# tum-vision/dvo_slam

Hardware: NVIDIA H100
Metric: frame-pair alignments/sec @640x480x5-level (higher is better)
Workload: dtype f32

## Files before the change

### dvo_slam_b200/csrc/capi.cu

```cuda
#include "common.cuh"

#include <cstdio>
#include <cstdlib>
#include <cstring>
#include <limits>
#include <vector>

namespace dvo_b200 {

int set_error(dvo_b200_ctx* ctx, int code, const std::string& msg) {
  if (ctx) ctx->last_error = msg;
  return code;
}

int check_cuda(dvo_b200_ctx* ctx, cudaError_t e, const char* what) {
  if (e == cudaSuccess) return 0;
  std::string msg = std::string("CUDA error: ") + cudaGetErrorString(e) + " in " + what;
  cudaGetLastError();
  return set_error(ctx, e == cudaErrorMemoryAllocation ? DVO_B200_ERR_OUT_OF_MEMORY : DVO_B200_ERR_CUDA, msg);
}

static cudaEvent_t get_event(dvo_b200_ctx* ctx) {
  if (!ctx->event_pool.empty()) { cudaEvent_t e = ctx->event_pool.back(); ctx->event_pool.pop_back(); return e; }
  cudaEvent_t e;
// ... 50 lines not shown
  if (cudaGetDeviceCount(&count) != cudaSuccess || count <= 0 || device < 0 || device >= count) {
    cudaGetLastError();
    return DVO_B200_ERR_CUDA;
  }
  if (cudaSetDevice(device) != cudaSuccess) { cudaGetLastError(); return DVO_B200_ERR_CUDA; }
  dvo_b200_ctx* ctx = new dvo_b200_ctx;
  ctx->device = device;
  ctx->pool = std::make_shared<SlabPool>();
  ctx->pool->device = device;
  if (stream) { ctx->stream = (cudaStream_t)stream; ctx->own_stream = false; }
  else {
    if (cudaStreamCreateWithFlags(&ctx->stream, cudaStreamNonBlocking) != cudaSuccess) { cudaGetLastError(); delete ctx; return DVO_B200_ERR_CUDA; }
    ctx->own_stream = true;
  }
  if (getenv("DVO_B200_TIMING")) {
    cudaMalloc((void**)&ctx->d_dbg, sizeof(unsigned long long) * 256);
    cudaMemset(ctx->d_dbg, 0, sizeof(unsigned long long) * 256);
    for (int l = 0; l < 8; ++l) { unsigned long long big = ~0ull; cudaMemcpy(ctx->d_dbg + 128 + 8 * l + 6, &big, 8, cudaMemcpyHostToDevice); }
  }
  *out = ctx;
  return 0;
}

int dvo_b200_destroy(dvo_b200_ctx* ctx) {
  if (!ctx) return DVO_B200_ERR_INVALID_ARGUMENT;
  cudaSetDevice(ctx->device);
  cudaStreamSynchronize(ctx->stream);
  drain_profile(ctx);
  for (cudaEvent_t e : ctx->event_pool) cudaEventDestroy(e);
  Workspace& ws = ctx->ws;
  cudaFree(ws.d_pair_level); cudaFree(ws.d_state); cudaFree(ws.d_row_exports); cudaFree(ws.d_row_base);
  cudaFree(ws.d_strip_exports); cudaFree(ws.d_strip_base); cudaFree(ws.d_row_partial); cudaFree(ws.d_strip_partial); cudaFree(ws.d_dump); cudaFree(ws.d_tinit);
// ... 234 lines not shown
  return tracker_linearize(ctx, cfg, reference, current, level, T, use_weights, prev_precision, count, precision_out, ll_out,
                           A_out, b_out, nullptr);
}

int dvo_b200_profile_enable(dvo_b200_ctx* ctx, int32_t enable) {
  if (!ctx) return DVO_B200_ERR_INVALID_ARGUMENT;
  ctx->profile = enable != 0;
  return 0;
}

int dvo_b200_profile_read(dvo_b200_ctx* ctx, double ms_out[8], int64_t launches_out[8], int32_t reset) {
  if (!ctx) return DVO_B200_ERR_INVALID_ARGUMENT;
  cudaSetDevice(ctx->device);
  drain_profile(ctx);
  if (ctx->d_dbg) {
    unsigned long long h[256];
    cudaStreamSynchronize(ctx->stream);
    cudaMemcpy(h, ctx->d_dbg, sizeof(h), cudaMemcpyDeviceToHost);
    static const char* names[8] = {"stageA", "stageB", "waitA", "waitB", "mid", "end", "queue", "total"};
    for (int l = 0; l < 8; ++l) {
      const unsigned long long* v = h + 16 * l;
      if (!v[7]) continue;
      fprintf(stderr, "[dvo_b200 timing] level-slot %d:", l);
      for (int i = 0; i < 8; ++i) fprintf(stderr, " %s=%.1f%%", names[i], 100.0 * (double)v[i] / (double)v[7]);
      fprintf(stderr, " (cta-ms total %.1f)\n", (double)v[7] * 1e-6);
      fprintf(stderr, "[dvo_b200 timing]   consumer warp 0: wait-full %.1f%% of stage A, %.1f%% of stage B; producer: descriptor %.1f%%, "
                      "wait-empty %.1f%% of its stage time\n", 100.0 * (double)v[9] / (double)(v[8] + 1), 100.0 * (double)v[11] / (double)(v[10] + 1),
              100.0 * (double)v[12] / (double)(v[14] + v[15] + 1), 100.0 * (double)v[13] / (double)(v[14] + v[15] + 1));
      const unsigned long long* u = h + 128 + 8 * l;
      if (u[0]) fprintf(stderr, "[dvo_b200 timing]   tiles %llu (inexact %.2f%%, skipped %.2f%%), stage-B rounds in the generic loop %.2f%%; CTA lifetime of the last launch-set: "
                                "max %.3f ms, min %.3f ms\n", u[0], 100.0 * (double)u[1] / (double)u[0], 100.0 * (double)u[2] / (double)u[0],
                        100.0 * (double)u[4] / (double)(u[3] + 1), (double)u[5] * 1e-6, (double)u[6] * 1e-6);
      const unsigned long long* e = h + 192 + 8 * l;
      if (e[7]) {
        double tot = 0;
        for (int i = 0; i < 6; ++i) tot += (double)e[i];
        fprintf(stderr, "[dvo_b200 timing]   end step: critical part %.1f%% of the end time; of the end thread's time: partial sums %.1f%%, state+log %.1f%%, "
                        "LDLT %.1f%%, exp+K*T %.1f%%, release %.1f%%, deferred %.1f%% (total %.1f cta-ms)\n", 100.0 * (double)e[7] / (double)(v[5] + 1),
                100.0 * e[0] / tot, 100.0 * e[1] / tot, 100.0 * e[2] / tot, 100.0 * e[3] / tot, 100.0 * e[4] / tot, 100.0 * e[5] / tot, tot * 1e-6);
      }
    }
    if (reset) {
      cudaMemset(ctx->d_dbg, 0, sizeof(h));
      for (int l = 0; l < 8; ++l) { unsigned long long big = ~0ull; cudaMemcpy(ctx->d_dbg + 128 + 8 * l + 6, &big, 8, cudaMemcpyHostToDevice); }
    }
  }
  if (getenv("DVO_B200_TIMING")) {
// ... 15 lines not shown
```

### dvo_slam_b200/csrc/stages.cuh

```cuda
#pragma once
#include "common.cuh"
#include "f32x2.cuh"

namespace dvo_b200 {

constexpr unsigned kFullMask = 0xffffffffu;
constexpr int kConsumerWarps = kTileH;
constexpr int kCtaThreads = (kConsumerWarps + 1) * 32;
#ifndef DVO_WIN_COLS
#define DVO_WIN_COLS 152
#endif
#ifndef DVO_WIN_ROWS
#define DVO_WIN_ROWS 24
#endif
#ifndef DVO_STAGES
#define DVO_STAGES 2
#endif
constexpr int kWinCols = DVO_WIN_COLS;
constexpr int kWinRows = DVO_WIN_ROWS;
constexpr int kStages = DVO_STAGES;

__device__ __forceinline__ unsigned smem_u32(const void* p) { return (unsigned)__cvta_generic_to_shared(p); }
__device__ __forceinline__ void mbar_init(unsigned long long* bar, unsigned count) {
  asm volatile("mbarrier.init.shared::cta.b64 [%0], %1;" ::"r"(smem_u32(bar)), "r"(count) : "memory");
}
__device__ __forceinline__ void mbar_fence_init() { asm volatile("fence.mbarrier_init.release.cluster;" ::: "memory"); }
__device__ __forceinline__ void mbar_arrive(unsigned long long* bar) {
  asm volatile("{\n\t.reg .b64 st;\n\tmbarrier.arrive.release.cta.shared::cta.b64 st, [%0];\n\t}" ::"r"(smem_u32(bar)) : "memory");
}
__device__ __forceinline__ void mbar_arrive_expect_tx(unsigned long long* bar, unsigned bytes) {
  asm volatile("{\n\t.reg .b64 st;\n\tmbarrier.arrive.expect_tx.release.cta.shared::cta.b64 st, [%0], %1;\n\t}" ::"r"(smem_u32(bar)),
               "r"(bytes)
               : "memory");
}
#ifndef DVO_TRYWAIT_HINT_NS
// ... 48 lines not shown
    if (((++spins) & 0xfffu) == 0u) {
      if (*reinterpret_cast<volatile int*>(error_flag)) break;
      if (spins > (1u << 24)) { atomicExch(error_flag, 2); break; }
    }
  }
}
__device__ __forceinline__ void mbar_arrive_s(unsigned bar) {
  asm volatile("{\n\t.reg .b64 st;\n\tmbarrier.arrive.release.cta.shared::cta.b64 st, [%0];\n\t}" ::"r"(bar) : "memory");
}
__device__ __forceinline__ int4 lds_i4(unsigned addr) {
  int4 v;
  asm volatile("ld.shared.v4.b32 {%0, %1, %2, %3}, [%4];" : "=r"(v.x), "=r"(v.y), "=r"(v.z), "=r"(v.w) : "r"(addr));
  return v;
}

__device__ __forceinline__ void bulk_g2s(void* dst_smem, const void* src_gmem, unsigned bytes, unsigned long long* bar) {
  asm volatile("cp.async.bulk.shared::cta.global.mbarrier::complete_tx::bytes [%0], [%1], %2, [%3];" ::"r"(smem_u32(dst_smem)),
               "l"(src_gmem), "r"(bytes), "r"(smem_u32(bar))
               : "memory");
}

template <int kOff>
__device__ __forceinline__ f2 lds_f2(unsigned addr) {
  f2 v;
  asm volatile("ld.shared.v2.f32 {%0, %1}, [%2+%3];" : "=f"(v.x), "=f"(v.y) : "r"(addr), "n"(kOff));
  return v;
}
__device__ __forceinline__ float lds_f32(unsigned addr) {
  float v;
  asm volatile("ld.shared.f32 %0, [%1];" : "=f"(v) : "r"(addr));
// ... 15 lines not shown
  int skip;
  int origin;
  int ulo, ucount;
  int vlo, vcount;
  int exact;
  int pad_;
};
struct __align__(128) StageBuf {
  float2 ref0[kTileH][kTileW];
  float tx[kTileW];
  float2 ref1[kTileH][kTileW];
  float2 win[kWinRows][kWinCols];
};
static_assert(offsetof(StageBuf, tx) == kRecTx * sizeof(float2) && offsetof(StageBuf, ref1) == kRecP1 * sizeof(float2) &&
              offsetof(StageBuf, win) == kRecF2 * sizeof(float2), "StageBuf must mirror the reference tile record");
struct TilePipe {
  StageBuf buf[kStages];
  unsigned long long full[kStages], empty[kStages];
  TileDesc desc[kStages];
};
static_assert(sizeof(TileDesc) == 32 && offsetof(TilePipe, desc) % 16 == 0, "TileDesc is read as two 16-byte words");

#ifdef DVO_PIPE_TIMING
struct PipeTiming {
  unsigned long long wait_full_a = 0, wait_full_b = 0, wait_empty = 0, produce = 0, rounds_a = 0, rounds_b = 0;
  unsigned long long tiles = 0, tiles_inexact = 0, tiles_skipped = 0, slow_rounds = 0, rounds = 0;
  bool on = false;
};
#define DVO_CLOCK(tm) ((tm).on ? clock64() : 0)
#define DVO_ADD(tm, field, v) do { if ((tm).on) (tm).field += (v); } while (0)
#else
struct PipeTiming {};
#define DVO_CLOCK(tm) 0ll
#define DVO_ADD(tm, field, v) do { } while (0)
#endif

struct LevelGeom {
  int w, h, n, pitch;
  int nbands, nstrips;
  int strip0, strip_step, nmine;
};
// ... 17 lines not shown
  c.k0 = pk(kt[0], kt[4]); c.k1 = pk(kt[1], kt[5]); c.k2 = pk(kt[2], kt[6]); c.k3 = pk(kt[3], kt[7]);
  c.k8 = kt[8]; c.k9 = kt[9]; c.k10 = kt[10]; c.k11 = kt[11];
  c.Pa = pk(P[0], P[1]); c.Pb = pk(P[2], P[3]);
  const float cgx = __fdiv_rn(__fmul_rn(0.5f, pl.cfx), 255.0f), cgy = __fdiv_rn(__fmul_rn(0.5f, pl.cfy), 255.0f);
  c.cg = pk(cgx, cgy);
  c.cgh = pk(0.5f * cgx, 0.5f * cgy);
  c.fxyh = pk(0.5f * pl.cfx, 0.5f * pl.cfy);
  c.c_i = 1.0f / 255.0f;
  c.ubx = pin((float)(w - 2)); c.uby = pin((float)(h - 2));
  c.first_iteration = __ldcg(&st.iteration) == 0;
}

template <bool kStageB>
__device__ __noinline__ void produce_tiles(TilePipe& tp, const PairLevel& pl, const LevelGeom& g, const StageConsts& c, unsigned tbase,
                                           int ntiles, int* error_flag, PipeTiming& tm) {
  const int lane = threadIdx.x & 31, sub = lane >> 3;
  const float2* cur = kStageB ? pl.c3 : pl.c0;
  int s_issue = g.strip0, b_issue = 0;
  for (int i0 = 0; i0 < ntiles; i0 += 4) {
    const long long tp0 = DVO_CLOCK(tm);
    unsigned wordA, wordD;
    {
      const int ii = min(i0 + sub, ntiles - 1);
      const int sd = ii / g.nbands;
      const int s = g.strip0 + sd * g.strip_step, b = ii - sd * g.nbands;
      const int y0 = s * kTileH, rows = min(kTileH, g.h - y0);
      const int x0 = b * kTileW, bw = min(kTileW, g.w - x0);
      const float2 zr = __ldg(pl.rrange + (size_t)s * g.nbands + b);
      const float txc = __ldg(pl.rtmpl + ((lane & 1) ? x0 + bw - 1 : x0));
      const float tyc = __ldg(pl.rtmpl + g.w + ((lane & 2) ? y0 + rows - 1 : y0));
      const bool has_depth = zr.x <= zr.y;
      const float z = (lane & 4) ? zr.y : zr.x;
      const float px = txc * z, py = tyc * z;
// ... 4 lines not shown
      const bool front_lane = Zt > 1e-6f && umin == umin && vmin == vmin;
#pragma unroll
      for (int off = 1; off < 8; off <<= 1) {
        umin = fminf(umin, __shfl_xor_sync(kFullMask, umin, off)); umax = fmaxf(umax, __shfl_xor_sync(kFullMask, umax, off));
        vmin = fminf(vmin, __shfl_xor_sync(kFullMask, vmin, off)); vmax = fmaxf(vmax, __shfl_xor_sync(kFullMask, vmax, off));
      }
      const bool front = ((__ballot_sync(kFullMask, front_lane) >> (sub * 8)) & 0xffu) == 0xffu;
      umin = fmaxf(umin, -8.f); vmin = fmaxf(vmin, -8.f); umax = fminf(umax, (float)g.w + 8.f); vmax = fminf(vmax, (float)g.h + 8.f);
      int skip = 0, exact = 0, ncols = 0, nrows = 0, bx0 = 0, row_lo = 0;
      if (!has_depth) {
        skip = 1;
      } else if (!front) {
      } else if (umax < -1.f || vmax < -1.f || umin > (float)g.w || vmin > (float)g.h) {
        skip = 1;
      } else {
        const int col_lo = max((int)floorf(umin) - 2, 0), col_hi = min((int)floorf(umax) + 3, g.w - 1);
        row_lo = max((int)floorf(vmin) - 2, -1);
        const int row_hi = min((int)floorf(vmax) + 3, g.h);
        bx0 = col_lo & ~1;
        ncols = (col_hi + 2 - bx0) & ~1;
        bool whole = true;
        if (ncols > kWinCols) { bx0 += ((ncols - kWinCols) / 2) & ~1; ncols = kWinCols; whole = false; }
        nrows = row_hi - row_lo + 1;
        if (nrows > kWinRows) { row_lo += (nrows - kWinRows) / 2; nrows = kWinRows; whole = false; }
        if (ncols < 4 || nrows < 4) { ncols = 0; nrows = 0; bx0 = 0; row_lo = 0; }
        else exact = whole ? 1 : 0;
      }
      wordA = (unsigned)skip | ((unsigned)exact << 1) | ((unsigned)ncols << 2) | ((unsigned)nrows << 10);
      wordD = (unsigned)bx0 | ((unsigned)(row_lo + 1) << 16);
    }
    DVO_ADD(tm, produce, DVO_CLOCK(tm) - tp0);
    const int kmax = min(4, ntiles - i0);
    for (int k = 0; k < kmax; ++k) {
      const unsigned t = tbase + (unsigned)(i0 + k);
      const int bufi = t % kStages;
      StageBuf& sb = tp.buf[bufi];
      const unsigned wa = __shfl_sync(kFullMask, wordA, k * 8), wd = __shfl_sync(kFullMask, wordD, k * 8);
      const int s = s_issue, b = b_issue;
      if (++b_issue == g.nbands) { b_issue = 0; s_issue += g.strip_step; }
      const int skip = (int)(wa & 1u), ncols = (int)((wa >> 2) & 0xffu), nrows = (int)(wa >> 10);
      const int win_bx0 = (int)(wd & 0xffffu), win_row_lo = (int)(wd >> 16) - 1;
      TileDesc d;
      d.skip = skip; d.exact = (int)((wa >> 1) & 1u); d.pad_ = 0;
      d.origin = 0; d.ulo = 0; d.ucount = 0; d.vlo = 0; d.vcount = 0;
      if (ncols) {
        d.origin = (win_row_lo * kWinCols + win_bx0) * 8;
        d.ulo = win_bx0 == 0 ? 0 : win_bx0 + 1;
        const int uhi = (win_bx0 + ncols - 1 >= g.w - 1) ? g.w - 2 : win_bx0 + ncols - 3;
        d.ucount = max(uhi - d.ulo + 1, 0);
        d.vlo = win_row_lo + 1;
        d.vcount = max(nrows - 3, 0);
      }
      const unsigned win_row_bytes = (unsigned)ncols * 8u;
      const unsigned rec_bytes = (unsigned)(kStageB ? kRecF2 : kRecP1) * 8u;
      const unsigned total = skip ? 0u : rec_bytes + (unsigned)nrows * win_row_bytes;
      const long long tp1 = DVO_CLOCK(tm);
      mbar_wait(&tp.empty[bufi], ((t / kStages) & 1u) ^ 1u, error_flag);
      DVO_ADD(tm, wait_empty, DVO_CLOCK(tm) - tp1);
      DVO_ADD(tm, tiles, 1); DVO_ADD(tm, tiles_inexact, (!d.skip && !d.exact) ? 1 : 0); DVO_ADD(tm, tiles_skipped, d.skip ? 1 : 0);
      if (lane == 0) {
        tp.desc[bufi] = d;
        if (total) mbar_arrive_expect_tx(&tp.full[bufi], total);
        else mbar_arrive(&tp.full[bufi]);
      }
      __syncwarp();
      if (!skip) {
        if (lane < nrows) {
          const int yy = min(max(win_row_lo + lane, 0), g.h - 1);
          bulk_g2s(&sb.win[lane][0], cur + (size_t)yy * g.pitch + win_bx0, win_row_bytes, &tp.full[bufi]);
        }
        if (lane == 31) bulk_g2s(&sb.ref0[0][0], pl.r0 + (size_t)(s * g.nbands + b) * kRecF2, rec_bytes, &tp.full[bufi]);
      }
    }
  }
}

struct PixelProjection {
  f2 f, gq;
  float Zt;
  int u0, v0;
  bool inb;
};

__device__ __forceinline__ PixelProjection project_pixel(float tx, float ty, float z, const StageConsts& c) {
  PixelProjection p;
  const f2 pxy = mul2(pk(tx, ty), bc(z));
// ... 344 lines not shown
  }
  if (lane == 0) {
    seg_out[0] = __int_as_float(st.cnt);
    seg_out[1] = (float)(0.5 * ((double)all0 + (double)alt0)); seg_out[2] = (float)(0.5 * ((double)all1 + (double)alt1));
    seg_out[3] = (float)(0.5 * ((double)all2 + (double)alt2));
    seg_out[4] = (float)(0.5 * ((double)all0 - (double)alt0)); seg_out[5] = (float)(0.5 * ((double)all1 - (double)alt1));
    seg_out[6] = (float)(0.5 * ((double)all2 - (double)alt2));
    seg_out[7] = st.wfirst;
    if (st.cnt == 0) { seg_out[8] = 0.f; seg_out[9] = 0.f; seg_out[10] = 0.f; seg_out[11] = 0.f; }
  }
  if (st.pend) {
    seg_out[8] = st.pw; seg_out[9] = st.po0; seg_out[10] = st.po1; seg_out[11] = st.po2;
  }
}

__device__ __forceinline__ WinView make_view(unsigned bufs, const int4& d0, const int4& d1, const float2* plane, int w, int h, int pitch) {
  WinView wv;
  const unsigned w0 = bufs + (unsigned)offsetof(StageBuf, win);
  wv.base = pin(w0 - (unsigned)d0.y);
  wv.safe = pin(w0 + (unsigned)((kWinCols + 1) * 8));
  wv.plane = plane;
  wv.exact = d1.z != 0;
  wv.ulo = d0.z; wv.ucount = d0.w; wv.vlo = d1.x; wv.vcount = d1.y;
  wv.w = w; wv.h = h; wv.pitch = pitch;
  return wv;
}


template <bool kCorrected, bool kExact, bool kFirst>
__device__ __forceinline__ void stage_a_rounds(const WinView& wv, int bw, unsigned refa, unsigned txa, float ty, const StageConsts& c,
                                               typename ScaleOf<kCorrected>::type& ss, int lane, unsigned lt_mask, int odd_col,
                                               float odd_z) {
  static_assert(kTileW % 64 == 0, "the exact loop takes whole pairs of rounds");
// ... 15 lines not shown
      z0 = (r * 32 + lane == odd_col) ? odd_z : z0;
      z1 = (r * 32 + 32 + lane == odd_col) ? odd_z : z1;
    }
    const PixelProjection p0 = project_pixel(tx0, ty, z0, c);
    const PixelProjection p1 = project_pixel(tx1, ty, z1, c);
    float ei0, ez0, ei1, ez1;
    const bool v0 = residual_pixel<kExact>(p0, wv, lo(rz0), z0, c, ei0, ez0);
    const bool v1 = residual_pixel<kExact>(p1, wv, lo(rz1), z1, c, ei1, ez1);
    const float w0 = student_weight(c, first, ei0, ez0), w1 = student_weight(c, first, ei1, ez1);
    scale_add(ss, lane, lt_mask, v0, w0, ei0, ez0);
    scale_add(ss, lane, lt_mask, v1, w1, ei1, ez1);
  }
}
template <bool kCorrected>
__device__ __forceinline__ void stage_a_run(TilePipe& tp, const PairLevel& pl, const LevelGeom& g, const StageConsts& c,
                                            float* row_exports, unsigned& tile_count, int* error_flag, PipeTiming& tm) {
  const int lane = threadIdx.x & 31, q = threadIdx.x >> 5;
  const unsigned lt_mask = (1u << lane) - 1u;
  const int ntiles = g.nmine * g.nbands;
  const unsigned tbase = tile_count;
  tile_count += ntiles;
  if (q == kConsumerWarps) {
    produce_tiles<false>(tp, pl, g, c, tbase, ntiles, error_flag, tm);
    return;
  }
  int i = 0;
  const unsigned tp_s = pin(smem_u32(&tp));
  const unsigned my_ref = pin((unsigned)(offsetof(StageBuf, ref0) + (q * kTileW + lane) * 8));
  const unsigned my_tx = pin((unsigned)(offsetof(StageBuf, tx) + lane * 4));
  const int gw = pin(g.w), gh = pin(g.h), gnb = pin(g.nbands), gpitch = g.pitch;
  OddPoint odd;
  odd.y = -1; odd.x = 0; odd.z = 0.f;
  if (kCorrected) odd = load_odd_point(pl, g);
  for (int sk = 0, s = g.strip0; sk < g.nmine; ++sk, s += g.strip_step) {
    const int y = s * kTileH + q;
    const bool row_ok = y < gh;
    const float ty = __ldg(pl.rtmpl + gw + min(y, gh - 1));
    typename ScaleOf<kCorrected>::type ss;
    scale_state_init(ss);
    for (int b = 0; b < gnb; ++b, ++i) {
      const unsigned t = tbase + i;
      const unsigned bufi = t % kStages;
      const int x0 = b * kTileW, bw = min(kTileW, gw - x0);
      const long long tw0 = DVO_CLOCK(tm);
      mbar_wait_s(tp_s + (unsigned)offsetof(TilePipe, full) + bufi * 8u, (t / kStages) & 1u, error_flag);
      DVO_ADD(tm, wait_full_a, DVO_CLOCK(tm) - tw0);
      const unsigned bufs = tp_s + bufi * (unsigned)sizeof(StageBuf);
      const int4 d0 = lds_i4(tp_s + (unsigned)offsetof(TilePipe, desc) + bufi * 32u);
      if (row_ok && !d0.x) {
        const int4 d1 = lds_i4(tp_s + (unsigned)offsetof(TilePipe, desc) + bufi * 32u + 16u);
        const WinView wv = make_view(bufs, d0, d1, pl.c0, gw, gh, gpitch);
        const unsigned refa = bufs + my_ref, txa = bufs + my_tx;
        const bool odd_tile = kCorrected && y == odd.y && (unsigned)(odd.x - x0) < (unsigned)bw;
        if (wv.exact && bw == kTileW && !odd_tile) {
          if (c.first_iteration) stage_a_rounds<kCorrected, true, true>(wv, bw, refa, txa, ty, c, ss, lane, lt_mask, -1, 0.f);
          else stage_a_rounds<kCorrected, true, false>(wv, bw, refa, txa, ty, c, ss, lane, lt_mask, -1, 0.f);
        } else {
          stage_a_rounds<kCorrected, false, false>(wv, bw, refa, txa, ty, c, ss, lane, lt_mask, odd_tile ? odd.x - x0 : -1, odd.z);
        }
      }
      __syncwarp();
      if (lane == 0) mbar_arrive_s(tp_s + (unsigned)offsetof(TilePipe, empty) + bufi * 8u);
    }
    if (row_ok) scale_state_export(ss, lane, row_exports + (size_t)y * kSegExportFloats);
  }
}

struct StageBConsts {
  float P00, P01, P10, P11;
  float l, wd0, wd1;
};

constexpr int kNormalValues = 28;

constexpr int kTriValues = 21;
__host__ __device__ constexpr int tri(int r, int c) { return r * 6 - r * (r - 1) / 2 + (c - r); }
struct StageBAcc {
// ... 118 lines not shown
      const unsigned m = __ballot_sync(kFullMask, valid);
      keep = valid && (rank + __popc(m & lt_mask)) < keep_rank;
      rank += __popc(m);
    }
    if (kDump && r * 32 < xlim) dump_record(dump, pix + r * 32, valid, E, G, H, z);
    const float ei = valid ? lo(E) : 0.f, ez = valid ? hi(E) : 0.f;
    const float wall = student_weight(c, first, ei, ez);
    const float wgt = valid ? wall : 0.f;
    stage_b_pixel(acc, cb, wgt, keep, ei, ez, valid ? G : bc(0.f), valid ? H : bc(0.f), valid ? z : 1.0f, valid ? tx : 0.f, ty);
  }
}

template <bool kDump, bool kCorrected>
__device__ __forceinline__ void stage_b_run(TilePipe& tp, const PairLevel& pl, const LevelGeom& g, const StageConsts& c,
                                            const StageBConsts& cb, const int* row_base, const int* strip_base, long long n_keep,
                                            const RecordDump& dump, float* row_partial, unsigned& tile_count, int* error_flag,
                                            PipeTiming& tm) {
  const int lane = threadIdx.x & 31, q = threadIdx.x >> 5;
  const unsigned lt_mask = (1u << lane) - 1u;
  const int ntiles = g.nmine * g.nbands;
  const unsigned tbase = tile_count;
  tile_count += ntiles;
  if (q == kConsumerWarps) {
    produce_tiles<true>(tp, pl, g, c, tbase, ntiles, error_flag, tm);
    return;
  }
  int i = 0;
  const unsigned tp_s = pin(smem_u32(&tp));
  const unsigned my_ref = (unsigned)(offsetof(StageBuf, ref0) + (q * kTileW + lane) * 8);
  const unsigned my_tx = (unsigned)(offsetof(StageBuf, tx) + lane * 4);
  const int gw = g.w, gh = g.h, gnb = g.nbands, gpitch = g.pitch;
  OddPoint odd;
  odd.y = -1; odd.x = 0; odd.z = 0.f;
  if (kCorrected) odd = load_odd_point(pl, g);
  for (int sk = 0, s = g.strip0; sk < g.nmine; ++sk, s += g.strip_step) {
    const int y = s * kTileH + q;
    const bool row_ok = y < gh;
// ... 2 lines not shown
    int keep_rank = 0;
    int rank = 0;
    if (!kCorrected) {
      const long long sbase = __ldcg(strip_base + s);
      cta_has_tail = (long long)__ldcg(strip_base + s + 1) > n_keep;
      keep_rank = (int)max(min(n_keep - sbase, (long long)0x7fffffff), (long long)-1);
      if (cta_has_tail && row_ok) rank = __ldcg(row_base + y);
    }
    StageBAcc acc;
    stage_b_init(acc);
    for (int b = 0; b < gnb; ++b, ++i) {
      const unsigned t = tbase + i;
      const unsigned bufi = t % kStages;
      const int x0 = b * kTileW, bw = min(kTileW, gw - x0);
      const long long tw0 = DVO_CLOCK(tm);
      mbar_wait_s(tp_s + (unsigned)offsetof(TilePipe, full) + bufi * 8u, (t / kStages) & 1u, error_flag);
      DVO_ADD(tm, wait_full_b, DVO_CLOCK(tm) - tw0);
      const unsigned bufs = tp_s + bufi * (unsigned)sizeof(StageBuf);
      const int4 d0 = lds_i4(tp_s + (unsigned)offsetof(TilePipe, desc) + bufi * 32u);
      if (row_ok && !d0.x) {
        const int4 d1 = lds_i4(tp_s + (unsigned)offsetof(TilePipe, desc) + bufi * 32u + 16u);
        const WinView wv = make_view(bufs, d0, d1, pl.c3, gw, gh, gpitch);
        const unsigned refa = bufs + my_ref, txa = bufs + my_tx;
        const size_t pix = (size_t)y * gw + x0 + lane;
        const bool odd_tile = kCorrected && y == odd.y && (unsigned)(odd.x - x0) < (unsigned)bw;
        if (wv.exact && bw == kTileW && !cta_has_tail && !odd_tile) {
          if (c.first_iteration)
            stage_b_rounds<kCorrected, true, true, kDump>(wv, bw, refa, txa, ty, c, cb, acc, cta_has_tail, rank, keep_rank, dump, pix, lane,
                                                          lt_mask, -1, 0.f, tm);
          else
            stage_b_rounds<kCorrected, true, false, kDump>(wv, bw, refa, txa, ty, c, cb, acc, cta_has_tail, rank, keep_rank, dump, pix, lane,
                                                           lt_mask, -1, 0.f, tm);
        } else {
          stage_b_rounds<kCorrected, false, false, kDump>(wv, bw, refa, txa, ty, c, cb, acc, cta_has_tail, rank, keep_rank, dump, pix, lane,
                                                          lt_mask, odd_tile ? odd.x - x0 : -1, odd.z, tm);
        }
      } else if (kDump && row_ok) {
        for (int xl = lane; xl < bw; xl += 32) dump_record(dump, (size_t)y * gw + x0 + xl, false, bc(0.f), bc(0.f), bc(0.f), 0.f);
      }
      __syncwarp();
      if (lane == 0) mbar_arrive_s(tp_s + (unsigned)offsetof(TilePipe, empty) + bufi * 8u);
    }
    if (row_ok) flush_row_partial(acc, lane, row_partial + (size_t)y * kNormalValues);
  }
}

__device__ __forceinline__ void load_stage_b_consts(const PairState& st, StageBConsts& c) {
  c.P00 = __ldcg(&st.precision[0]); c.P01 = __ldcg(&st.precision[1]); c.P10 = __ldcg(&st.precision[2]); c.P11 = __ldcg(&st.precision[3]);
  c.l = c.P01 / c.P00;
  c.wd0 = c.P00;
  c.wd1 = c.P11 - c.P01 * c.l;
}

}
```

### dvo_slam_b200/csrc/tracker.cu

```cuda
#include "common.cuh"
#include "stages.cuh"

#include <cstdio>
#include <cstring>
#include <limits>
#include <cmath>
#include <cstdlib>
#include <algorithm>

namespace dvo_b200 {

namespace {

constexpr unsigned kFull = 0xffffffffu;
constexpr int kEndWarps = 4;

struct LevelLaunch {
  int w, h, n, pitch;
  int nbands, nstrips;
  int level_index;
  int level_id;
  int max_iterations;
  int first_level;
  int use_initial_estimate;
// ... 252 lines not shown
}

struct SquadState {
  int pair;
  unsigned arrive;
  unsigned phase;
  int pad_[29];
};

struct LevelTail {
  SegCombineSmem comb;
  PairEndSmem end;
  int s_flag[2];
};
constexpr size_t kLevelSmemBytes = sizeof(TilePipe) + sizeof(LevelTail);

constexpr int kMaxSeg = 4;
struct Segment {
  const PairLevel* pls;
  float* row_exports;
  int* row_base;
  double* strip_exports;
  int* strip_base;
  float* row_partial;
  double* strip_partial;
  SquadState* squads;
  int* queue;
  int* ready;
  int* ready_tail;
  int* arrivals;
// ... 61 lines not shown
    }
  }
  __syncthreads();
}

template <bool kCorrected>
__global__ void __launch_bounds__(kCtaThreads, 2)
k_level_persistent(const __grid_constant__ PersistentArgs a) {
  extern __shared__ __align__(128) unsigned char smem_raw[];
  TilePipe& tp = *reinterpret_cast<TilePipe*>(smem_raw);
  LevelTail& lt = *reinterpret_cast<LevelTail*>(smem_raw + sizeof(TilePipe));

  const int warp = threadIdx.x >> 5, lane = threadIdx.x & 31;

  if (threadIdx.x == 0) {
    for (int i = 0; i < kStages; ++i) { mbar_init(&tp.full[i], 1); mbar_init(&tp.empty[i], kConsumerWarps); }
    mbar_fence_init();
  }
  __syncthreads();
  unsigned tile_count = 0;
  const bool fused = a.nseg >= 2;
#define DVO_TICK() do { if (timing) t0 = global_ns(); } while (0)
#define DVO_TOCK(slot) do { if (timing) { t1 = global_ns(); t_acc[slot] += t1 - t0; t0 = t1; } } while (0)

#pragma unroll 1
  for (int si = 0; si < a.nseg; ++si) {
  const Segment& S = a.seg[si];
  int cta_index = blockIdx.x;
  if (fused && si >= 1) {
    if (threadIdx.x == 0) lt.s_flag[1] = atomicAdd(S.arrivals, 1);
    __syncthreads();
    cta_index = lt.s_flag[1];
    __syncthreads();
  }
  const int squad = cta_index / S.g, rank = cta_index - squad * S.g;
// ... 68 lines not shown
          squad_release(sq, episode);
        }
      } else {
        squad_wait(sq, episode, a.error_flag);
      }
      __syncthreads();
      ++episode;
      DVO_TOCK(6);
    }

    for (;;) {
      {
        StageConsts c;
        load_stage_consts(st, pl, lp.w, lp.h, false, c);
        const long long ts0 = DVO_CLOCK(tm);
        stage_a_run<kCorrected>(tp, pl, geo, c, row_exports, tile_count, a.error_flag, tm);
        DVO_ADD(tm, rounds_a, DVO_CLOCK(tm) - ts0);
      }
      __syncthreads();
      for (int j = threadIdx.x; j < geo.nmine; j += kCtaThreads) {
        const int sj = geo.strip0 + j * geo.strip_step;
        combine_strip_rows(row_exports, sj * kTileH, min(sj * kTileH + kTileH, lp.h), row_base, strip_exports + (size_t)sj * kStripExportDoubles);
      }
      DVO_TOCK(0);
      if (squad_arrive(sq, episode, S.g, lt.s_flag)) {
        DVO_TOCK(2);
        if (warp == 0) {
          pair_mid_warp<kCorrected>(st, pair, strip_exports, strip_base, lp.nstrips, nullptr, lp, a.ilog, a.max_log, lt.comb);
          if (lane == 0) squad_release(sq, episode);
        }
        __syncthreads();
// ... 3 lines not shown
        DVO_TOCK(2);
      }
      __syncthreads();
      ++episode;
      if (!__ldcg(&st.level_active) || *reinterpret_cast<volatile int*>(a.error_flag)) break;

      {
        StageConsts c;
        load_stage_consts(st, pl, lp.w, lp.h, true, c);
        StageBConsts cb;
        load_stage_b_consts(st, cb);
        const long long n_keep = __ldcg(&st.n_keep);
        RecordDump dump;
        dump.planes = a.dump; dump.n = lp.n;
        const long long ts0 = DVO_CLOCK(tm);
        if (a.dump) stage_b_run<true, kCorrected>(tp, pl, geo, c, cb, row_base, strip_base, n_keep, dump, row_partial, tile_count, a.error_flag, tm);
        else stage_b_run<false, kCorrected>(tp, pl, geo, c, cb, row_base, strip_base, n_keep, dump, row_partial, tile_count, a.error_flag, tm);
        DVO_ADD(tm, rounds_b, DVO_CLOCK(tm) - ts0);
      }
      __syncthreads();
      for (int it = threadIdx.x; it < geo.nmine * kNormalValues; it += kCtaThreads) {
        const int j = it / kNormalValues, i = it - j * kNormalValues;
        const int sj = geo.strip0 + j * geo.strip_step;
        const int nrow = min(kTileH, lp.h - sj * kTileH);
        const float* rp = row_partial + (size_t)sj * kTileH * kNormalValues + i;
        float r[kTileH];
#pragma unroll
        for (int k = 0; k < kTileH; ++k) r[k] = k < nrow ? __ldcg(rp + (size_t)k * kNormalValues) : 0.f;
        double v = 0.0;
#pragma unroll
        for (int k = 0; k < kTileH; ++k) v += (double)r[k];
        strip_partial[(size_t)sj * kNormalValues + i] = v;
// ... 20 lines not shown
      __threadfence();
      const int slot = atomicAdd(a.seg[k].ready_tail, 1);
      asm volatile("st.release.gpu.global.u32 [%0], %1;" :: "l"(a.seg[k].ready + slot), "r"(pair + 1) : "memory");
    }
  }
  if (timing) {
    t_acc[7] = global_ns() - t_start;
    for (int i = 0; i < 8; ++i) atomicAdd(S.dbg + i, t_acc[i]);
  }
#ifdef DVO_PIPE_TIMING
  if (tm.on) {
    if (warp == 0) { atomicAdd(S.dbg + 8, tm.rounds_a); atomicAdd(S.dbg + 9, tm.wait_full_a); atomicAdd(S.dbg + 10, tm.rounds_b); atomicAdd(S.dbg + 11, tm.wait_full_b); }
    else { atomicAdd(S.dbg + 12, tm.produce); atomicAdd(S.dbg + 13, tm.wait_empty); atomicAdd(S.dbg + 14, tm.rounds_a); atomicAdd(S.dbg + 15, tm.rounds_b); }
    if (warp == 0) { atomicAdd(S.dbg2 + 3, tm.rounds); atomicAdd(S.dbg2 + 4, tm.slow_rounds); }
    else { atomicAdd(S.dbg2 + 0, tm.tiles); atomicAdd(S.dbg2 + 1, tm.tiles_inexact); atomicAdd(S.dbg2 + 2, tm.tiles_skipped); }
  }
  if (timing) { atomicMax(S.dbg2 + 5, t_acc[7]); atomicMin(S.dbg2 + 6, t_acc[7]); }
#endif
  }
#undef DVO_TICK
#undef DVO_TOCK
}

__global__ void k_finalize(PairState* states, dvo_b200_result* results, int npairs) {
  int p = blockIdx.x * blockDim.x + threadIdx.x;
  if (p >= npairs) return;
  PairState& st = states[p];
  dvo_b200_result& r = results[p];
  const double nan = __longlong_as_double(0x7ff8000000000000LL);
  se3_matrix(se3_inverse(st.estimate), r.transformation);
// ... 560 lines not shown
```

Measured before the change: 21140.

## Give stage A its own smaller-window, deeper tile ring sharing stage B's smem

Splits the tile pipeline into separate stage-A and stage-B rings that share one shared-memory union. Stage A gets a 16-row window with no third gradient record, a tighter halo and three slots, so its producer can prefetch further ahead. Stage B keeps its 2-slot, 24-row layout. Each stage now has its own barriers, descriptors and tile counters, and a proxy fence is added before the bulk copies reuse the slots. The change also adds timing counters for stage A, and any stage-A tile whose footprint exceeds 16 rows falls off the exact path more often.

```diff
diff --git a/dvo_slam_b200/csrc/capi.cu b/dvo_slam_b200/csrc/capi.cu
--- a/dvo_slam_b200/csrc/capi.cu
+++ b/dvo_slam_b200/csrc/capi.cu
@@ -88,8 +88,8 @@
     ctx->own_stream = true;
   }
   if (getenv("DVO_B200_TIMING")) {
-    cudaMalloc((void**)&ctx->d_dbg, sizeof(unsigned long long) * 256);
-    cudaMemset(ctx->d_dbg, 0, sizeof(unsigned long long) * 256);
+    cudaMalloc((void**)&ctx->d_dbg, sizeof(unsigned long long) * 320);
+    cudaMemset(ctx->d_dbg, 0, sizeof(unsigned long long) * 320);
     for (int l = 0; l < 8; ++l) { unsigned long long big = ~0ull; cudaMemcpy(ctx->d_dbg + 128 + 8 * l + 6, &big, 8, cudaMemcpyHostToDevice); }
   }
   *out = ctx;
@@ -354,7 +354,7 @@
   cudaSetDevice(ctx->device);
   drain_profile(ctx);
   if (ctx->d_dbg) {
-    unsigned long long h[256];
+    unsigned long long h[320];
     cudaStreamSynchronize(ctx->stream);
     cudaMemcpy(h, ctx->d_dbg, sizeof(h), cudaMemcpyDeviceToHost);
     static const char* names[8] = {"stageA", "stageB", "waitA", "waitB", "mid", "end", "queue", "total"};
@@ -371,6 +371,10 @@
       if (u[0]) fprintf(stderr, "[dvo_b200 timing]   tiles %llu (inexact %.2f%%, skipped %.2f%%), stage-B rounds in the generic loop %.2f%%; CTA lifetime of the last launch-set: "
                                 "max %.3f ms, min %.3f ms\n", u[0], 100.0 * (double)u[1] / (double)u[0], 100.0 * (double)u[2] / (double)u[0],
                         100.0 * (double)u[4] / (double)(u[3] + 1), (double)u[5] * 1e-6, (double)u[6] * 1e-6);
+      const unsigned long long* a = h + 256 + 8 * l;
+      if (a[1]) fprintf(stderr, "[dvo_b200 timing]   stage A: tiles %llu (inexact %.2f%%, skipped %.2f%%), producer wait-empty %.1f%% of its stage-A time; "
+                                "stage B: producer wait-empty %.1f%% of its stage-B time\n", a[1], 100.0 * (double)a[2] / (double)a[1],
+                        100.0 * (double)a[3] / (double)a[1], 100.0 * (double)a[0] / (double)(v[14] + 1), 100.0 * (double)(v[13] - a[0]) / (double)(v[15] + 1));
       const unsigned long long* e = h + 192 + 8 * l;
       if (e[7]) {
         double tot = 0;
diff --git a/dvo_slam_b200/csrc/stages.cuh b/dvo_slam_b200/csrc/stages.cuh
--- a/dvo_slam_b200/csrc/stages.cuh
+++ b/dvo_slam_b200/csrc/stages.cuh
@@ -16,9 +16,17 @@
 #ifndef DVO_STAGES
 #define DVO_STAGES 2
 #endif
+#ifndef DVO_WIN_ROWS_A
+#define DVO_WIN_ROWS_A 16
+#endif
+#ifndef DVO_STAGES_A
+#define DVO_STAGES_A 3
+#endif
 constexpr int kWinCols = DVO_WIN_COLS;
 constexpr int kWinRows = DVO_WIN_ROWS;
 constexpr int kStages = DVO_STAGES;
+constexpr int kWinRowsA = DVO_WIN_ROWS_A;
+constexpr int kStagesA = DVO_STAGES_A;
 
 __device__ __forceinline__ unsigned smem_u32(const void* p) { return (unsigned)__cvta_generic_to_shared(p); }
 __device__ __forceinline__ void mbar_init(unsigned long long* bar, unsigned count) {
@@ -97,6 +105,8 @@
   return v;
 }
 
+__device__ __forceinline__ void fence_proxy_async_smem() { asm volatile("fence.proxy.async.shared::cta;" ::: "memory"); }
+
 __device__ __forceinline__ void bulk_g2s(void* dst_smem, const void* src_gmem, unsigned bytes, unsigned long long* bar) {
   asm volatile("cp.async.bulk.shared::cta.global.mbarrier::complete_tx::bytes [%0], [%1], %2, [%3];" ::"r"(smem_u32(dst_smem)),
                "l"(src_gmem), "r"(bytes), "r"(smem_u32(bar))
@@ -142,17 +152,33 @@
 };
 static_assert(offsetof(StageBuf, tx) == kRecTx * sizeof(float2) && offsetof(StageBuf, ref1) == kRecP1 * sizeof(float2) &&
               offsetof(StageBuf, win) == kRecF2 * sizeof(float2), "StageBuf must mirror the reference tile record");
+struct __align__(128) StageBufA {
+  float2 ref0[kTileH][kTileW];
+  float tx[kTileW];
+  float2 win[kWinRowsA][kWinCols];
+};
+static_assert(offsetof(StageBufA, tx) == kRecTx * sizeof(float2) && offsetof(StageBufA, win) == kRecP1 * sizeof(float2),
+              "StageBufA must mirror the reference tile record up to the gradient rows");
+static_assert(sizeof(StageBuf) % 128 == 0 && sizeof(StageBufA) % 128 == 0, "slots start on 128-byte boundaries");
 struct TilePipe {
-  StageBuf buf[kStages];
-  unsigned long long full[kStages], empty[kStages];
-  TileDesc desc[kStages];
-};
-static_assert(sizeof(TileDesc) == 32 && offsetof(TilePipe, desc) % 16 == 0, "TileDesc is read as two 16-byte words");
+  union {
+    StageBuf b[kStages];
+    StageBufA a[kStagesA];
+  } ring;
+  TileDesc descA[kStagesA], descB[kStages];
+  unsigned long long fullA[kStagesA], emptyA[kStagesA], fullB[kStages], emptyB[kStages];
+};
+static_assert(offsetof(TilePipe, ring) == 0, "slot addresses are the pipe's address plus slot * slot size");
+static_assert(kStagesA * sizeof(StageBufA) <= sizeof(TilePipe::ring) && kStages * sizeof(StageBuf) <= sizeof(TilePipe::ring),
+              "both layouts fit the shared ring");
+static_assert(sizeof(TileDesc) == 32 && offsetof(TilePipe, descA) % 16 == 0 && offsetof(TilePipe, descB) % 16 == 0,
+              "TileDesc is read as two 16-byte words");
 
 #ifdef DVO_PIPE_TIMING
 struct PipeTiming {
   unsigned long long wait_full_a = 0, wait_full_b = 0, wait_empty = 0, produce = 0, rounds_a = 0, rounds_b = 0;
   unsigned long long tiles = 0, tiles_inexact = 0, tiles_skipped = 0, slow_rounds = 0, rounds = 0;
+  unsigned long long wait_empty_a = 0, tiles_a = 0, tiles_inexact_a = 0, tiles_skipped_a = 0;
   bool on = false;
 };
 #define DVO_CLOCK(tm) ((tm).on ? clock64() : 0)
@@ -200,9 +226,14 @@
 template <bool kStageB>
 __device__ __noinline__ void produce_tiles(TilePipe& tp, const PairLevel& pl, const LevelGeom& g, const StageConsts& c, unsigned tbase,
                                            int ntiles, int* error_flag, PipeTiming& tm) {
+  constexpr int kS = kStageB ? kStages : kStagesA, kRows = kStageB ? kWinRows : kWinRowsA;
+  unsigned long long* const full = kStageB ? tp.fullB : tp.fullA;
+  unsigned long long* const empty = kStageB ? tp.emptyB : tp.emptyA;
+  TileDesc* const desc = kStageB ? tp.descB : tp.descA;
   const int lane = threadIdx.x & 31, sub = lane >> 3;
   const float2* cur = kStageB ? pl.c3 : pl.c0;
   int s_issue = g.strip0, b_issue = 0;
+  fence_proxy_async_smem();
   for (int i0 = 0; i0 < ntiles; i0 += 4) {
     const long long tp0 = DVO_CLOCK(tm);
     unsigned wordA, wordD;
@@ -237,15 +268,16 @@
       } else if (umax < -1.f || vmax < -1.f || umin > (float)g.w || vmin > (float)g.h) {
         skip = 1;
       } else {
-        const int col_lo = max((int)floorf(umin) - 2, 0), col_hi = min((int)floorf(umax) + 3, g.w - 1);
-        row_lo = max((int)floorf(vmin) - 2, -1);
-        const int row_hi = min((int)floorf(vmax) + 3, g.h);
+        constexpr int kLo = kStageB ? 2 : 1, kHi = kStageB ? 3 : 2;
+        const int col_lo = max((int)floorf(umin) - kLo, 0), col_hi = min((int)floorf(umax) + kHi, g.w - 1);
+        row_lo = max((int)floorf(vmin) - kLo, kStageB ? -1 : 0);
+        const int row_hi = min((int)floorf(vmax) + kHi, kStageB ? g.h : g.h - 1);
         bx0 = col_lo & ~1;
         ncols = (col_hi + 2 - bx0) & ~1;
         bool whole = true;
         if (ncols > kWinCols) { bx0 += ((ncols - kWinCols) / 2) & ~1; ncols = kWinCols; whole = false; }
         nrows = row_hi - row_lo + 1;
-        if (nrows > kWinRows) { row_lo += (nrows - kWinRows) / 2; nrows = kWinRows; whole = false; }
+        if (nrows > kRows) { row_lo += (nrows - kRows) / 2; nrows = kRows; whole = false; }
         if (ncols < 4 || nrows < 4) { ncols = 0; nrows = 0; bx0 = 0; row_lo = 0; }
         else exact = whole ? 1 : 0;
       }
@@ -256,8 +288,9 @@
     const int kmax = min(4, ntiles - i0);
     for (int k = 0; k < kmax; ++k) {
       const unsigned t = tbase + (unsigned)(i0 + k);
-      const int bufi = t % kStages;
-      StageBuf& sb = tp.buf[bufi];
+      const int bufi = t % kS;
+      float2* const rec = kStageB ? &tp.ring.b[bufi].ref0[0][0] : &tp.ring.a[bufi].ref0[0][0];
+      float2* const win = kStageB ? &tp.ring.b[bufi].win[0][0] : &tp.ring.a[bufi].win[0][0];
       const unsigned wa = __shfl_sync(kFullMask, wordA, k * 8), wd = __shfl_sync(kFullMask, wordD, k * 8);
       const int s = s_issue, b = b_issue;
       if (++b_issue == g.nbands) { b_issue = 0; s_issue += g.strip_step; }
@@ -268,31 +301,41 @@
       d.origin = 0; d.ulo = 0; d.ucount = 0; d.vlo = 0; d.vcount = 0;
       if (ncols) {
         d.origin = (win_row_lo * kWinCols + win_bx0) * 8;
-        d.ulo = win_bx0 == 0 ? 0 : win_bx0 + 1;
-        const int uhi = (win_bx0 + ncols - 1 >= g.w - 1) ? g.w - 2 : win_bx0 + ncols - 3;
-        d.ucount = max(uhi - d.ulo + 1, 0);
-        d.vlo = win_row_lo + 1;
-        d.vcount = max(nrows - 3, 0);
+        if (kStageB) {
+          d.ulo = win_bx0 == 0 ? 0 : win_bx0 + 1;
+          const int uhi = (win_bx0 + ncols - 1 >= g.w - 1) ? g.w - 2 : win_bx0 + ncols - 3;
+          d.ucount = max(uhi - d.ulo + 1, 0);
+          d.vlo = win_row_lo + 1;
+          d.vcount = max(nrows - 3, 0);
+        } else {
+          d.ulo = win_bx0; d.ucount = ncols - 1;
+          d.vlo = win_row_lo; d.vcount = nrows - 1;
+        }
       }
       const unsigned win_row_bytes = (unsigned)ncols * 8u;
       const unsigned rec_bytes = (unsigned)(kStageB ? kRecF2 : kRecP1) * 8u;
       const unsigned total = skip ? 0u : rec_bytes + (unsigned)nrows * win_row_bytes;
       const long long tp1 = DVO_CLOCK(tm);
-      mbar_wait(&tp.empty[bufi], ((t / kStages) & 1u) ^ 1u, error_flag);
-      DVO_ADD(tm, wait_empty, DVO_CLOCK(tm) - tp1);
+      mbar_wait(&empty[bufi], ((t / kS) & 1u) ^ 1u, error_flag);
+      const long long tp2 = DVO_CLOCK(tm);
+      DVO_ADD(tm, wait_empty, tp2 - tp1);
       DVO_ADD(tm, tiles, 1); DVO_ADD(tm, tiles_inexact, (!d.skip && !d.exact) ? 1 : 0); DVO_ADD(tm, tiles_skipped, d.skip ? 1 : 0);
+      if (!kStageB) {
+        DVO_ADD(tm, wait_empty_a, tp2 - tp1);
+        DVO_ADD(tm, tiles_a, 1); DVO_ADD(tm, tiles_inexact_a, (!d.skip && !d.exact) ? 1 : 0); DVO_ADD(tm, tiles_skipped_a, d.skip ? 1 : 0);
+      }
       if (lane == 0) {
-        tp.desc[bufi] = d;
-        if (total) mbar_arrive_expect_tx(&tp.full[bufi], total);
-        else mbar_arrive(&tp.full[bufi]);
+        desc[bufi] = d;
+        if (total) mbar_arrive_expect_tx(&full[bufi], total);
+        else mbar_arrive(&full[bufi]);
       }
       __syncwarp();
       if (!skip) {
         if (lane < nrows) {
           const int yy = min(max(win_row_lo + lane, 0), g.h - 1);
-          bulk_g2s(&sb.win[lane][0], cur + (size_t)yy * g.pitch + win_bx0, win_row_bytes, &tp.full[bufi]);
+          bulk_g2s(win + lane * kWinCols, cur + (size_t)yy * g.pitch + win_bx0, win_row_bytes, &full[bufi]);
         }
-        if (lane == 31) bulk_g2s(&sb.ref0[0][0], pl.r0 + (size_t)(s * g.nbands + b) * kRecF2, rec_bytes, &tp.full[bufi]);
+        if (lane == 31) bulk_g2s(rec, pl.r0 + (size_t)(s * g.nbands + b) * kRecF2, rec_bytes, &full[bufi]);
       }
     }
   }
@@ -667,9 +710,11 @@
   }
 }
 
+template <typename Buf>
 __device__ __forceinline__ WinView make_view(unsigned bufs, const int4& d0, const int4& d1, const float2* plane, int w, int h, int pitch) {
+  static_assert(2 * kWinCols * sizeof(float2) + 2 * sizeof(float2) <= sizeof(Buf::win), "`safe` taps lie inside the slot's window");
   WinView wv;
-  const unsigned w0 = bufs + (unsigned)offsetof(StageBuf, win);
+  const unsigned w0 = bufs + (unsigned)offsetof(Buf, win);
   wv.base = pin(w0 - (unsigned)d0.y);
   wv.safe = pin(w0 + (unsigned)((kWinCols + 1) * 8));
   wv.plane = plane;
@@ -715,20 +760,20 @@
 }
 template <bool kCorrected>
 __device__ __forceinline__ void stage_a_run(TilePipe& tp, const PairLevel& pl, const LevelGeom& g, const StageConsts& c,
-                                            float* row_exports, unsigned& tile_count, int* error_flag, PipeTiming& tm) {
+                                            float* row_exports, unsigned& tile_count_a, int* error_flag, PipeTiming& tm) {
   const int lane = threadIdx.x & 31, q = threadIdx.x >> 5;
   const unsigned lt_mask = (1u << lane) - 1u;
   const int ntiles = g.nmine * g.nbands;
-  const unsigned tbase = tile_count;
-  tile_count += ntiles;
+  const unsigned tbase = tile_count_a;
+  tile_count_a += ntiles;
   if (q == kConsumerWarps) {
     produce_tiles<false>(tp, pl, g, c, tbase, ntiles, error_flag, tm);
     return;
   }
   int i = 0;
   const unsigned tp_s = pin(smem_u32(&tp));
-  const unsigned my_ref = pin((unsigned)(offsetof(StageBuf, ref0) + (q * kTileW + lane) * 8));
-  const unsigned my_tx = pin((unsigned)(offsetof(StageBuf, tx) + lane * 4));
+  const unsigned my_ref = pin((unsigned)(offsetof(StageBufA, ref0) + (q * kTileW + lane) * 8));
+  const unsigned my_tx = pin((unsigned)(offsetof(StageBufA, tx) + lane * 4));
   const int gw = pin(g.w), gh = pin(g.h), gnb = pin(g.nbands), gpitch = g.pitch;
   OddPoint odd;
   odd.y = -1; odd.x = 0; odd.z = 0.f;
@@ -741,16 +786,16 @@
     scale_state_init(ss);
     for (int b = 0; b < gnb; ++b, ++i) {
       const unsigned t = tbase + i;
-      const unsigned bufi = t % kStages;
+      const unsigned bufi = t % kStagesA;
       const int x0 = b * kTileW, bw = min(kTileW, gw - x0);
       const long long tw0 = DVO_CLOCK(tm);
-      mbar_wait_s(tp_s + (unsigned)offsetof(TilePipe, full) + bufi * 8u, (t / kStages) & 1u, error_flag);
+      mbar_wait_s(tp_s + (unsigned)offsetof(TilePipe, fullA) + bufi * 8u, (t / kStagesA) & 1u, error_flag);
       DVO_ADD(tm, wait_full_a, DVO_CLOCK(tm) - tw0);
-      const unsigned bufs = tp_s + bufi * (unsigned)sizeof(StageBuf);
-      const int4 d0 = lds_i4(tp_s + (unsigned)offsetof(TilePipe, desc) + bufi * 32u);
+      const unsigned bufs = tp_s + bufi * (unsigned)sizeof(StageBufA);
+      const int4 d0 = lds_i4(tp_s + (unsigned)offsetof(TilePipe, descA) + bufi * 32u);
       if (row_ok && !d0.x) {
-        const int4 d1 = lds_i4(tp_s + (unsigned)offsetof(TilePipe, desc) + bufi * 32u + 16u);
-        const WinView wv = make_view(bufs, d0, d1, pl.c0, gw, gh, gpitch);
+        const int4 d1 = lds_i4(tp_s + (unsigned)offsetof(TilePipe, descA) + bufi * 32u + 16u);
+        const WinView wv = make_view<StageBufA>(bufs, d0, d1, pl.c0, gw, gh, gpitch);
         const unsigned refa = bufs + my_ref, txa = bufs + my_tx;
         const bool odd_tile = kCorrected && y == odd.y && (unsigned)(odd.x - x0) < (unsigned)bw;
         if (wv.exact && bw == kTileW && !odd_tile) {
@@ -761,7 +806,7 @@
         }
       }
       __syncwarp();
-      if (lane == 0) mbar_arrive_s(tp_s + (unsigned)offsetof(TilePipe, empty) + bufi * 8u);
+      if (lane == 0) mbar_arrive_s(tp_s + (unsigned)offsetof(TilePipe, emptyA) + bufi * 8u);
     }
     if (row_ok) scale_state_export(ss, lane, row_exports + (size_t)y * kSegExportFloats);
   }
@@ -910,13 +955,13 @@
 template <bool kDump, bool kCorrected>
 __device__ __forceinline__ void stage_b_run(TilePipe& tp, const PairLevel& pl, const LevelGeom& g, const StageConsts& c,
                                             const StageBConsts& cb, const int* row_base, const int* strip_base, long long n_keep,
-                                            const RecordDump& dump, float* row_partial, unsigned& tile_count, int* error_flag,
+                                            const RecordDump& dump, float* row_partial, unsigned& tile_count_b, int* error_flag,
                                             PipeTiming& tm) {
   const int lane = threadIdx.x & 31, q = threadIdx.x >> 5;
   const unsigned lt_mask = (1u << lane) - 1u;
   const int ntiles = g.nmine * g.nbands;
-  const unsigned tbase = tile_count;
-  tile_count += ntiles;
+  const unsigned tbase = tile_count_b;
+  tile_count_b += ntiles;
   if (q == kConsumerWarps) {
     produce_tiles<true>(tp, pl, g, c, tbase, ntiles, error_flag, tm);
     return;
@@ -949,13 +994,13 @@
       const unsigned bufi = t % kStages;
       const int x0 = b * kTileW, bw = min(kTileW, gw - x0);
       const long long tw0 = DVO_CLOCK(tm);
-      mbar_wait_s(tp_s + (unsigned)offsetof(TilePipe, full) + bufi * 8u, (t / kStages) & 1u, error_flag);
+      mbar_wait_s(tp_s + (unsigned)offsetof(TilePipe, fullB) + bufi * 8u, (t / kStages) & 1u, error_flag);
       DVO_ADD(tm, wait_full_b, DVO_CLOCK(tm) - tw0);
       const unsigned bufs = tp_s + bufi * (unsigned)sizeof(StageBuf);
-      const int4 d0 = lds_i4(tp_s + (unsigned)offsetof(TilePipe, desc) + bufi * 32u);
+      const int4 d0 = lds_i4(tp_s + (unsigned)offsetof(TilePipe, descB) + bufi * 32u);
       if (row_ok && !d0.x) {
-        const int4 d1 = lds_i4(tp_s + (unsigned)offsetof(TilePipe, desc) + bufi * 32u + 16u);
-        const WinView wv = make_view(bufs, d0, d1, pl.c3, gw, gh, gpitch);
+        const int4 d1 = lds_i4(tp_s + (unsigned)offsetof(TilePipe, descB) + bufi * 32u + 16u);
+        const WinView wv = make_view<StageBuf>(bufs, d0, d1, pl.c3, gw, gh, gpitch);
         const unsigned refa = bufs + my_ref, txa = bufs + my_tx;
         const size_t pix = (size_t)y * gw + x0 + lane;
         const bool odd_tile = kCorrected && y == odd.y && (unsigned)(odd.x - x0) < (unsigned)bw;
@@ -974,7 +1019,7 @@
         for (int xl = lane; xl < bw; xl += 32) dump_record(dump, (size_t)y * gw + x0 + xl, false, bc(0.f), bc(0.f), bc(0.f), 0.f);
       }
       __syncwarp();
-      if (lane == 0) mbar_arrive_s(tp_s + (unsigned)offsetof(TilePipe, empty) + bufi * 8u);
+      if (lane == 0) mbar_arrive_s(tp_s + (unsigned)offsetof(TilePipe, emptyB) + bufi * 8u);
     }
     if (row_ok) flush_row_partial(acc, lane, row_partial + (size_t)y * kNormalValues);
   }
diff --git a/dvo_slam_b200/csrc/tracker.cu b/dvo_slam_b200/csrc/tracker.cu
--- a/dvo_slam_b200/csrc/tracker.cu
+++ b/dvo_slam_b200/csrc/tracker.cu
@@ -290,6 +290,7 @@
   int s_flag[2];
 };
 constexpr size_t kLevelSmemBytes = sizeof(TilePipe) + sizeof(LevelTail);
+static_assert(2 * (kLevelSmemBytes + 1024) <= 228 * 1024, "two CTAs per SM: 228 KB of shared memory, 1 KB reserved per CTA");
 
 constexpr int kMaxSeg = 4;
 struct Segment {
@@ -381,11 +382,12 @@
   const int warp = threadIdx.x >> 5, lane = threadIdx.x & 31;
 
   if (threadIdx.x == 0) {
-    for (int i = 0; i < kStages; ++i) { mbar_init(&tp.full[i], 1); mbar_init(&tp.empty[i], kConsumerWarps); }
+    for (int i = 0; i < kStagesA; ++i) { mbar_init(&tp.fullA[i], 1); mbar_init(&tp.emptyA[i], kConsumerWarps); }
+    for (int i = 0; i < kStages; ++i) { mbar_init(&tp.fullB[i], 1); mbar_init(&tp.emptyB[i], kConsumerWarps); }
     mbar_fence_init();
   }
   __syncthreads();
-  unsigned tile_count = 0;
+  unsigned tile_count_a = 0, tile_count_b = 0;
   const bool fused = a.nseg >= 2;
 #define DVO_TICK() do { if (timing) t0 = global_ns(); } while (0)
 #define DVO_TOCK(slot) do { if (timing) { t1 = global_ns(); t_acc[slot] += t1 - t0; t0 = t1; } } while (0)
@@ -484,7 +486,7 @@
         StageConsts c;
         load_stage_consts(st, pl, lp.w, lp.h, false, c);
         const long long ts0 = DVO_CLOCK(tm);
-        stage_a_run<kCorrected>(tp, pl, geo, c, row_exports, tile_count, a.error_flag, tm);
+        stage_a_run<kCorrected>(tp, pl, geo, c, row_exports, tile_count_a, a.error_flag, tm);
         DVO_ADD(tm, rounds_a, DVO_CLOCK(tm) - ts0);
       }
       __syncthreads();
@@ -518,8 +520,8 @@
         RecordDump dump;
         dump.planes = a.dump; dump.n = lp.n;
         const long long ts0 = DVO_CLOCK(tm);
-        if (a.dump) stage_b_run<true, kCorrected>(tp, pl, geo, c, cb, row_base, strip_base, n_keep, dump, row_partial, tile_count, a.error_flag, tm);
-        else stage_b_run<false, kCorrected>(tp, pl, geo, c, cb, row_base, strip_base, n_keep, dump, row_partial, tile_count, a.error_flag, tm);
+        if (a.dump) stage_b_run<true, kCorrected>(tp, pl, geo, c, cb, row_base, strip_base, n_keep, dump, row_partial, tile_count_b, a.error_flag, tm);
+        else stage_b_run<false, kCorrected>(tp, pl, geo, c, cb, row_base, strip_base, n_keep, dump, row_partial, tile_count_b, a.error_flag, tm);
         DVO_ADD(tm, rounds_b, DVO_CLOCK(tm) - ts0);
       }
       __syncthreads();
@@ -570,6 +572,10 @@
     else { atomicAdd(S.dbg + 12, tm.produce); atomicAdd(S.dbg + 13, tm.wait_empty); atomicAdd(S.dbg + 14, tm.rounds_a); atomicAdd(S.dbg + 15, tm.rounds_b); }
     if (warp == 0) { atomicAdd(S.dbg2 + 3, tm.rounds); atomicAdd(S.dbg2 + 4, tm.slow_rounds); }
     else { atomicAdd(S.dbg2 + 0, tm.tiles); atomicAdd(S.dbg2 + 1, tm.tiles_inexact); atomicAdd(S.dbg2 + 2, tm.tiles_skipped); }
+    if (warp == kConsumerWarps) {
+      atomicAdd(S.dbg2 + 128, tm.wait_empty_a); atomicAdd(S.dbg2 + 129, tm.tiles_a); atomicAdd(S.dbg2 + 130, tm.tiles_inexact_a);
+      atomicAdd(S.dbg2 + 131, tm.tiles_skipped_a);
+    }
   }
   if (timing) { atomicMax(S.dbg2 + 5, t_acc[7]); atomicMin(S.dbg2 + 6, t_acc[7]); }
 #endif
```

New measurement: 21310, median of 6. Within noise of the previous version (+0.8%).
